# HunterJ-Lin/WSOVOD

Hardware: AMD Instinct MI355X
Metric: images/sec (512 proposals/img) WSR_18_DC5 fwd+bwd at 1/2/4/8 MI355X (higher is better)
Workload: dtype bf16 / fp16 + MX fp8 (the parity forward with the res4 / res5 convs and fc1 / fc2 on fp16 hi*hi + block-scaled e4m3 cross terms -- two v_mfma_f32_32x32x16_f16 + one v_mfma_scale_f32_32x32x64_f8f6f4 per 32x32x32 tile --, bf16x2 three-product forward elsewhere; plain bf16 backward; fp32 accumulation

## Files before the change

### include/wsovod_hip.h

```cpp
#ifndef WSOVOD_HIP_H_
#define WSOVOD_HIP_H_

#ifdef __cplusplus
extern "C" {
#endif

typedef void* wsovod_stream_t;

typedef enum {
  WSOVOD_OK = 0,
  WSOVOD_ERR_INVALID_ARGUMENT = 1,
  WSOVOD_ERR_HIP = 2,
  WSOVOD_ERR_UNSUPPORTED = 3
} wsovod_status;

typedef enum { WSOVOD_F32 = 0, WSOVOD_BF16 = 1, WSOVOD_BF16X2 = 2, WSOVOD_BF16X2P = 3, WSOVOD_F16MX = 4 } wsovod_dtype;
typedef enum { WSOVOD_NCHW = 0, WSOVOD_NHWC = 1 } wsovod_layout;

const char* wsovod_last_error(void);
int wsovod_abi_version(void);

typedef struct {
  const char* name;
  long long launches;
// ... 199 lines not shown
int wsovod_gemm_tn(const void* P, long long ldp, const void* Q, long long ldq, int Mred, int NI, int NJ, float* C,
                   long long ldc, float alpha, int accumulate, wsovod_stream_t stream);
int wsovod_gemm_tn_ex(const void* P, long long ldp, const void* Q, long long ldq, int q_dtype, int Mred, int NI, int NJ,
                      float* C, long long ldc, float alpha, int accumulate, wsovod_stream_t stream);
typedef struct wsovod_tn_sgd {
  float* param;
  float* momentum_buf;
  void* shadow;
  int shadow_is_bf16x2;
  float lr, weight_decay, momentum, grad_scale;
  const float* lr_dev;
  const unsigned char* mx_scale;
} wsovod_tn_sgd;
int wsovod_gemm_tn_sgd(const void* P, long long ldp, const void* Q, long long ldq, int q_dtype, int Mred, int NI, int NJ,
                       float alpha, const wsovod_tn_sgd* update, wsovod_stream_t stream);

int wsovod_f16mx_encode(const float* src, long long ld_src, int rows, int cols, int nseg, void* dst, long long ld_dst,
                        unsigned char* scales, wsovod_stream_t stream);
int wsovod_f16mx_encode_with(const float* src, long long ld_src, int rows, int cols, void* dst, long long ld_dst,
                             unsigned char* scales, const unsigned char* tensor_scale, wsovod_stream_t stream);
int wsovod_f16mx_from_bf16x2(const void* src, void* dst, long long n, wsovod_stream_t stream);
int wsovod_gemm_f16mx(const wsovod_gemm_desc* d, const unsigned char* a_scale, int a_segments, const unsigned char* b_scale,
                      int b_segments, void* c_bf16, long long ld_c_bf16, wsovod_stream_t stream);

typedef struct {
  int n_branch;
  int dil[4], pad[4];
  int shared_input;
} wsovod_conv_branches;
int wsovod_gemm_conv_branches(const wsovod_gemm_desc* d, const wsovod_conv_branches* br, wsovod_stream_t stream);
// ... 73 lines not shown
```

### wsovod_amd/_lib.py

```python
import ctypes as C
import os

import torch

_HERE = os.path.dirname(os.path.abspath(__file__))
LIB_PATH = os.path.join(_HERE, "lib", "libwsovod_hip.so")

F32, BF16, BF16X2, BF16X2P, F16MX = 0, 1, 2, 3, 4
NCHW, NHWC = 0, 1


class ConvGeom(C.Structure):
    _fields_ = [(n, C.c_int) for n in
                ("n_img", "H", "W", "Cin", "Ho", "Wo", "KH", "KW", "stride", "pad", "dil", "pool")]


class GemmDesc(C.Structure):
    _fields_ = [
        ("dtype_in", C.c_int), ("M", C.c_int), ("N", C.c_int), ("K", C.c_int),
        ("A", C.c_void_p), ("lda", C.c_longlong),
        ("B", C.c_void_p), ("ldb", C.c_longlong),
        ("C", C.c_void_p), ("ldc", C.c_longlong), ("dtype_c", C.c_int),
        ("Ct", C.c_void_p), ("ldct", C.c_longlong), ("dtype_ct", C.c_int),
        ("alpha", C.c_float),
# ... 74 lines not shown
    "wsovod_subsample_labels": [_P, _P, _P, _I, _I, _I, _I, _L, _P, _P],
    "wsovod_sgd_momentum_multi": [_P, _I, _F, _F, _P],
    "wsovod_grad_clip_workspace_floats": [_P, _I],
    "wsovod_grad_clip_coef": [_P, _I, _F, _F, _I, _P, _P, _P],
    "wsovod_roi_pool_workspace_bytes": [_I, _I, _I, _I, _I, _I, _I, _I, _I, _I],
    "wsovod_roi_pool_forward_ws": [_P, _I, _I, _P, _P, _I, _I, _I, _I, _I, _I, _I, _F, _P, _I, _P, _P, _P, _L, _P],
    "wsovod_roi_pool_forward_m2": [_P, _I, _I, _P, _P, _I, _I, _I, _I, _I, _I, _I, _F, _P, _I, _P, _P, _P, _L, _P],
    "wsovod_max2x2_gap_workspace_floats": [_I, _I, _I, _I, _I],
    "wsovod_max2x2_gap_nhwc": [_P, _I, _I, _I, _I, _I, _P, _P, _P, _P],
    "wsovod_pack_bf16_multi": [_P, _I, _P],
    "wsovod_sum_shards_bf16": [_P, _I, _L, _P, _P],
    "wsovod_format_rois": [_P, _P, _I, _I, _P, _P, _P, _P],
    "wsovod_gemm_tn": [_P, _L, _P, _L, _I, _I, _I, _P, _L, _F, _I, _P],
    "wsovod_gemm_tn_ex": [_P, _L, _P, _L, _I, _I, _I, _I, _P, _L, _F, _I, _P],
    "wsovod_gemm_tn_sgd": [_P, _L, _P, _L, _I, _I, _I, _I, _F, _P, _P],
    "wsovod_f16mx_encode": [_P, _L, _I, _I, _I, _P, _L, _P, _P],
    "wsovod_f16mx_encode_with": [_P, _L, _I, _I, _P, _L, _P, _P, _P],
    "wsovod_f16mx_from_bf16x2": [_P, _P, _L, _P],
    "wsovod_gemm_f16mx": [_P, _P, _I, _P, _I, _P, _L, _P],
    "wsovod_gemm_conv_branches": [C.POINTER(GemmDesc), C.POINTER(ConvBranches), _P],
    "wsovod_gemm_f16mx_conv_branches": [C.POINTER(GemmDesc), C.POINTER(ConvBranches), _P, _I, _P],
    "wsovod_mask_transpose_ex": [_P, _L, _I, _P, _L, _I, _I, _I, _F, _P, _L, _P, _L, _I, _P, _P],
    "wsovod_bf16x2_encode": [_P, _L, _I, _I, _P, _L, _P],
    "wsovod_bf16x2_decode": [_P, _L, _I, _I, _P, _L, _P],
    "wsovod_mask_bf16x2": [_P, _L, _P, _L, _I, _I, _I, _F, _P, _L, _P, _L, _P, _P],
    "wsovod_bf16x2_encode_t": [_P, _L, _I, _I, _P, _L, _P],
    "wsovod_f16mx_to_f32": [_P, _L, _I, _I, _P, _L, _P],
    "wsovod_f16mx_range": [_P, _L, _I, _I, _P, _P],
    "wsovod_stem_conv1_x2": [_P, _P, _P, _P, _I, _I, _I, _P, _P, _P, _P],
    "wsovod_nms_segments": [_P, _P, _P, _I, _I, _I, _F, _I, _P, _P, _P, _P],
# ... 104 lines not shown
```

### wsovod_amd/csrc/gemm_tn8.hip

```cpp
#include "gemm_common.h"
#include "f16mx.h"
#include <vector>

namespace wsovod_gemm {

namespace {

typedef __attribute__((ext_vector_type(4))) unsigned int u32x4;
typedef __attribute__((ext_vector_type(2))) unsigned int u32x2;

struct TnArgs {
  const char* P;
  const char* Q;
  long long ldp, ldq;
  int Mred, NI, NJ;
  float* C;
  long long ldc;
  float alpha;
  int accumulate;
  int tiles_i, tiles_j, group_m;
  int full_tiles, ksplit, slice_steps;
  float* partial;
#if defined(TN_STAMPS)
  float* dbg;
#endif
  int q_x2;
  float* mom;
  bf16_t* shadow;
  int shadow_x2;
  const unsigned char* mx_scale;
  float lr, wd, mu, gscale;
  const float* lr_dev;
  float* tail_buf;
  int bid_base;
};

template <int OFF>
__device__ __forceinline__ void tr_read_imm(__attribute__((ext_vector_type(2))) unsigned int& dst, unsigned addr) {
#if defined(__HIP_DEVICE_COMPILE__)
  asm volatile("ds_read_b64_tr_b16 %0, %1 offset:%2" : "=v"(dst) : "v"(addr), "n"(OFF));
#endif
}

template <int LEAN, bool SGD = false, bool TAILBUF = false>
__global__ __launch_bounds__(512) void gemm_tn8_kernel(const TnArgs p) {
  constexpr int BI = 256, BJ = 256, BK = 64;
  constexpr int OP_BYTES = 2 * BK * 256;
  constexpr int STEP_BYTES = 2 * OP_BYTES;
  constexpr int BUF_STRIDE = LEAN ? OP_BYTES : STEP_BYTES, OPQ_BASE = LEAN == 2 ? 2 * 5 * 8192 : LEAN ? 2 * OP_BYTES : OP_BYTES;
  constexpr int REG = 5 * 32 * 256;
  constexpr int SUB_STRIDE = LEAN == 2 ? REG : BK * 256;
  extern __shared__ __attribute__((aligned(16))) char smem[];

  int wg, slice = 0;
  const int bid = TAILBUF ? (int)blockIdx.x + p.bid_base : (int)blockIdx.x;
  {
    const int nwg = p.ksplit ? p.full_tiles : p.tiles_i * p.tiles_j;
    if (bid < nwg) {
      const int q = nwg >> 3, r = nwg & 7, xcd = bid & 7;
      wg = (xcd < r ? xcd * (q + 1) : r * (q + 1) + (xcd - r) * q) + (bid >> 3);
    } else {
      const int t = bid - nwg;
      wg = nwg + t / p.ksplit;
      slice = t - (t / p.ksplit) * p.ksplit;
    }
  }
  const bool sliced = p.ksplit && bid >= p.full_tiles;
  const int group_size = p.group_m * p.tiles_j;
  const int group_id = wg / group_size;
  const int first_i = group_id * p.group_m;
// ... 278 lines not shown
  if (sliced) {
    constexpr int SROW = 64;
    float* stg = (float*)smem + wave * (64 * SROW);
    const int cbase = j0 + wc * 64;
#pragma unroll
    for (int half = 0; half < 2; ++half) {
#pragma unroll
      for (int i = 0; i < 4; ++i)
#pragma unroll
        for (int j = 0; j < 4; ++j)
          *(f32x4*)(stg + (i * 16 + frow) * SROW + (((j * 4 + fq) ^ frow) << 2)) = acc[half * 4 + i][j] * p.alpha;
      __builtin_amdgcn_fence(__ATOMIC_RELEASE, "wavefront");
      __builtin_amdgcn_wave_barrier();
      const int rbase = i0 + wr * 128 + half * 64;
      const long long blk = (long long)(wr * 128 + half * 64) * 256 + wc * 64;
      float* dst = TAILBUF ? p.tail_buf + (long long)(wg - p.full_tiles) * 65536 + blk
                           : p.partial + ((long long)(wg - p.full_tiles) * p.ksplit + slice) * 65536 + blk;
      for (int row = 0; row < 64; ++row) {
        if (rbase + row >= p.NI) break;
        const float v = stg[row * SROW + ((((lane >> 2) ^ (row & 15)) << 2) | (lane & 3))];
        if (cbase + lane < p.NJ) {
          if constexpr (TAILBUF) unsafeAtomicAdd(dst + row * 256 + lane, v);
          else dst[row * 256 + lane] = v;
        }
      }
      __builtin_amdgcn_fence(__ATOMIC_ACQUIRE, "wavefront");
      __builtin_amdgcn_wave_barrier();
    }
    return;
  }
  if constexpr (SGD) {
    constexpr int SROW = 64;
    float* stg = (float*)smem + wave * (64 * SROW);
    const float lr = p.lr_dev ? *p.lr_dev : p.lr;
    const float ag = p.alpha, gs = p.gscale, mu = p.mu, wd = p.wd;
    const int mx_exp = p.shadow_x2 == 2 ? (int)*p.mx_scale - 127 : 0;
    const float mx_iq = __builtin_ldexpf(1.0f, -mx_exp), mx_il = __builtin_ldexpf(1.0f, -(mx_exp - 11));
    const int cbase = j0 + wc * 64;
    const int rsub = lane >> 4, c4 = (lane & 15) << 2;
#pragma unroll
    for (int half = 0; half < 2; ++half) {
#pragma unroll
      for (int i = 0; i < 4; ++i)
#pragma unroll
        for (int j = 0; j < 4; ++j)
          *(f32x4*)(stg + (i * 16 + frow) * SROW + (((j * 4 + fq) ^ frow) << 2)) = acc[half * 4 + i][j];
      __builtin_amdgcn_fence(__ATOMIC_RELEASE, "wavefront");
      __builtin_amdgcn_wave_barrier();
      const int rbase = i0 + wr * 128 + half * 64;
      if (cbase + c4 < p.NJ) {
#pragma unroll 4
        for (int it = 0; it < 16; ++it) {
          const int row = it * 4 + rsub;
          if (rbase + row >= p.NI) break;
          f32x4 gv = *(const f32x4*)(stg + row * SROW + ((((c4 >> 2)) ^ (row & 15)) << 2));
          const long long e = (long long)(rbase + row) * p.ldc + cbase + c4;
          f32x4 pv = __builtin_nontemporal_load((const f32x4*)(p.C + e));
          f32x4 bv = __builtin_nontemporal_load((const f32x4*)(p.mom + e));
          gv = gv * ag;
          gv = gv * gs;
          bv = mu * bv + (gv + wd * pv);
          pv -= lr * bv;
          __builtin_nontemporal_store(bv, (f32x4*)(p.mom + e));
          __builtin_nontemporal_store(pv, (f32x4*)(p.C + e));
          if (p.shadow && p.shadow_x2 == 2) {
            wsovod_mx::f16x4 h4;
            int q4, l4;
            wsovod_mx::mx_enc4(pv, mx_iq, mx_il, h4, q4, l4);
            char* grp = (char*)p.shadow + ((e >> 5) << 7);
            const int w = (int)(e & 31);
            *(wsovod_mx::f16x4*)(grp + 2 * w) = h4;
            *(int*)(grp + 64 + w) = q4;
            *(int*)(grp + 96 + w) = l4;
          } else if (p.shadow) {
            const bf16x4 hi = bf16x4{(bf16_t)pv[0], (bf16_t)pv[1], (bf16_t)pv[2], (bf16_t)pv[3]};
            if (p.shadow_x2) {
              bf16_t* q = p.shadow + ((e >> 5) << 6) + (e & 31);
              *(bf16x4*)q = hi;
              *(bf16x4*)(q + 32) = bf16x4{(bf16_t)(pv[0] - (float)hi[0]), (bf16_t)(pv[1] - (float)hi[1]),
                                          (bf16_t)(pv[2] - (float)hi[2]), (bf16_t)(pv[3] - (float)hi[3])};
            } else {
              *(bf16x4*)(p.shadow + e) = hi;
            }
          }
        }
      }
      __builtin_amdgcn_fence(__ATOMIC_ACQUIRE, "wavefront");
      __builtin_amdgcn_wave_barrier();
    }
    return;
  }
  const bool vec = (p.ldc & 3) == 0 && ((uintptr_t)p.C & 15) == 0 && j0 + BJ <= p.NJ;
#define WS_TN_ROW(I)                                                                                      \
  {                                                                                                       \
    const int ii = i0 + wr * 128 + (I) * 16 + frow;                                                       \
    if (ii < p.NI) {                                                                                      \
      float* crow = p.C + (long long)ii * p.ldc + j0 + wc * 64 + fq * 4;                                  \
// ... 34 lines not shown
    if (i >= p.NI) break;
    if (j >= p.NJ) continue;
    f32x4 acc = *(const f32x4*)(src + r * 256 + c4);
    for (int z = 1; z < nslices; ++z) acc += *(const f32x4*)(src + (long long)z * 65536 + r * 256 + c4);
    float* c = p.C + (long long)i * p.ldc + j;
    if (vec) {
      if (p.accumulate) acc += *(const f32x4*)c;
      *(f32x4*)c = acc;
    } else {
#pragma unroll
      for (int q = 0; q < 4; ++q) c[q] = p.accumulate ? c[q] + acc[q] : acc[q];
    }
  }
}

__global__ __launch_bounds__(256) void tn_sgd_tail_kernel(const TnArgs p) {
  const int wg = p.full_tiles + (blockIdx.x >> 4), part = blockIdx.x & 15;
  const int group_size = p.group_m * p.tiles_j;
  const int group_id = wg / group_size;
  const int first_i = group_id * p.group_m;
  const int gm = min(p.tiles_i - first_i, p.group_m);
  const int in_group = wg - group_id * group_size;
  const int i0 = (first_i + in_group % gm) * 256 + part * 16, j0 = (in_group / gm) * 256;
  const float* src = p.tail_buf + (long long)(wg - p.full_tiles) * 65536 + (long long)part * 16 * 256;
  const float lr = p.lr_dev ? *p.lr_dev : p.lr;
  const float gs = p.gscale, mu = p.mu, wd = p.wd;
  for (int e = threadIdx.x; e < 16 * 64; e += 256) {
    const int r = e >> 6, c4 = (e & 63) * 4;
    const int i = i0 + r, j = j0 + c4;
    if (i >= p.NI) break;
    if (j >= p.NJ) continue;
    f32x4 gv = *(const f32x4*)(src + r * 256 + c4);
    const long long q = (long long)i * p.ldc + j;
    f32x4 pv = *(const f32x4*)(p.C + q);
    f32x4 bv = *(const f32x4*)(p.mom + q);
    gv = gv * gs;
    bv = mu * bv + (gv + wd * pv);
    pv -= lr * bv;
    *(f32x4*)(p.mom + q) = bv;
    *(f32x4*)(p.C + q) = pv;
    if (p.shadow && p.shadow_x2 == 2) {
      const int mx_exp = (int)*p.mx_scale - 127;
      wsovod_mx::f16x4 h4;
      int q4, l4;
      wsovod_mx::mx_enc4(pv, __builtin_ldexpf(1.0f, -mx_exp), __builtin_ldexpf(1.0f, -(mx_exp - 11)), h4, q4, l4);
      char* grp = (char*)p.shadow + ((q >> 5) << 7);
      const int w = (int)(q & 31);
      *(wsovod_mx::f16x4*)(grp + 2 * w) = h4;
      *(int*)(grp + 64 + w) = q4;
      *(int*)(grp + 96 + w) = l4;
    } else if (p.shadow) {
      const bf16x4 hi = bf16x4{(bf16_t)pv[0], (bf16_t)pv[1], (bf16_t)pv[2], (bf16_t)pv[3]};
      if (p.shadow_x2) {
        bf16_t* d = p.shadow + ((q >> 5) << 6) + (q & 31);
        *(bf16x4*)d = hi;
        *(bf16x4*)(d + 32) = bf16x4{(bf16_t)(pv[0] - (float)hi[0]), (bf16_t)(pv[1] - (float)hi[1]),
                                    (bf16_t)(pv[2] - (float)hi[2]), (bf16_t)(pv[3] - (float)hi[3])};
      } else {
        *(bf16x4*)(p.shadow + q) = hi;
      }
    }
  }
}

}
}

static int tn_launch(const void* P, long long ldp, const void* Q, long long ldq, int q_dtype, int Mred, int NI, int NJ,
                     float* C, long long ldc, float alpha, int accumulate, const wsovod_tn_sgd* upd, wsovod_stream_t stream);

extern "C" int wsovod_gemm_tn_ex(const void* P, long long ldp, const void* Q, long long ldq, int q_dtype, int Mred, int NI,
                                 int NJ, float* C, long long ldc, float alpha, int accumulate, wsovod_stream_t stream) {
  return tn_launch(P, ldp, Q, ldq, q_dtype, Mred, NI, NJ, C, ldc, alpha, accumulate, nullptr, stream);
}

extern "C" int wsovod_gemm_tn_sgd(const void* P, long long ldp, const void* Q, long long ldq, int q_dtype, int Mred, int NI,
                                  int NJ, float alpha, const wsovod_tn_sgd* upd, wsovod_stream_t stream) {
  WS_CHECK_ARG(upd && upd->param && upd->momentum_buf, "wsovod_gemm_tn_sgd: null parameter / momentum buffer");
  WS_CHECK_ARG((((uintptr_t)upd->param | (uintptr_t)upd->momentum_buf) & 15) == 0 && ((uintptr_t)upd->shadow & 7) == 0,
               "wsovod_gemm_tn_sgd: parameter / momentum buffer must be 16-byte aligned (shadow: 8)");
  WS_CHECK_ARG(!upd->shadow || !upd->shadow_is_bf16x2 || NJ % 32 == 0,
               "wsovod_gemm_tn_sgd: a bf16x2 / f16mx shadow needs rows of whole 32-value groups");
  WS_CHECK_ARG(!upd->shadow || upd->shadow_is_bf16x2 != 2 || (upd->mx_scale && ((uintptr_t)upd->shadow & 15) == 0),
               "wsovod_gemm_tn_sgd: an f16mx shadow needs its per-tensor scale byte and 16-byte alignment");
  return tn_launch(P, ldp, Q, ldq, q_dtype, Mred, NI, NJ, upd->param, NJ, alpha, 2, upd, stream);
}

extern "C" int wsovod_gemm_tn(const void* P, long long ldp, const void* Q, long long ldq, int Mred, int NI, int NJ,
                              float* C, long long ldc, float alpha, int accumulate, wsovod_stream_t stream) {
  return wsovod_gemm_tn_ex(P, ldp, Q, ldq, WSOVOD_BF16, Mred, NI, NJ, C, ldc, alpha, accumulate, stream);
}

static int tn_launch(const void* P, long long ldp, const void* Q, long long ldq, int q_dtype, int Mred, int NI, int NJ,
                     float* C, long long ldc, float alpha, int accumulate, const wsovod_tn_sgd* upd, wsovod_stream_t stream) {
  using namespace wsovod_gemm;
  WS_CHECK_ARG(q_dtype == WSOVOD_BF16 || q_dtype == WSOVOD_BF16X2, "wsovod_gemm_tn: Q must be bf16 or bf16x2");
  const bool q_x2 = q_dtype == WSOVOD_BF16X2;
  WS_CHECK_ARG(!q_x2 || (NJ % 32 == 0 && ldq % 4 == 0), "wsovod_gemm_tn: a bf16x2 Q needs NJ a multiple of 32");
  if (q_x2) ldq *= 2;
  WS_CHECK_ARG(Mred >= 0 && NI >= 0 && NJ >= 0, "wsovod_gemm_tn: negative dimension");
  if (NI == 0 || NJ == 0) return WSOVOD_OK;
  WS_CHECK_ARG(P && Q && C, "wsovod_gemm_tn: null pointer");
  WS_CHECK_ARG((((uintptr_t)P | (uintptr_t)Q) & 15) == 0, "wsovod_gemm_tn: P/Q must be 16-byte aligned");
  WS_CHECK_ARG(ldp % 8 == 0 && ldq % 8 == 0 && NI % 8 == 0 && NJ % 8 == 0,
               "wsovod_gemm_tn: row strides and column counts must be multiples of 8 bf16 elements");
  WS_CHECK_ARG((long long)Mred * ldp * 2 < (1ll << 31) && (long long)Mred * ldq * 2 < (1ll << 31),
               "wsovod_gemm_tn: operand exceeds the 2 GiB buffer-addressing limit");
  TnArgs a;
  a.P = (const char*)P;
// ... 3 lines not shown
  a.Mred = Mred;
  a.NI = NI;
  a.NJ = NJ;
  a.C = C;
  a.ldc = ldc;
  a.alpha = alpha;
  a.accumulate = accumulate & 1;
  a.q_x2 = q_x2 ? 1 : 0;
  a.mom = nullptr;
  a.shadow = nullptr;
  a.shadow_x2 = 0;
  a.mx_scale = nullptr;
  a.lr = a.wd = a.mu = 0.f;
  a.gscale = 1.f;
  a.lr_dev = nullptr;
  a.tail_buf = nullptr;
  a.bid_base = 0;
  if (upd) {
    a.mom = upd->momentum_buf;
    a.shadow = (bf16_t*)upd->shadow;
    a.shadow_x2 = upd->shadow_is_bf16x2;
    a.mx_scale = upd->mx_scale;
    a.lr = upd->lr;
    a.wd = upd->weight_decay;
    a.mu = upd->momentum;
    a.gscale = upd->grad_scale;
    a.lr_dev = upd->lr_dev;
  }
#if defined(TN_STAMPS)
  a.dbg = getenv("WSOVOD_TN_DEBUG_PTR") ? (float*)strtoull(getenv("WSOVOD_TN_DEBUG_PTR"), nullptr, 16) : nullptr;
#endif
  a.tiles_i = ceil_div(NI, 256);
// ... 2 lines not shown
    const int run = std::max(1, a.tiles_i * a.tiles_j / 8);
    int g = 1;
    while ((g + 1) * (g + 1) <= run) ++g;
    a.group_m = std::max(1, std::min(std::min(g, 8), a.tiles_i));
  }
  static int slot_plain = wsovod::prof_slot("gemm_tn_bf16_256x256_tr");
  static int slot_sgd = wsovod::prof_slot("gemm_tn_bf16_256x256_tr_sgd");
  const int slot = upd ? slot_sgd : slot_plain;
  static bool attr_set = false;
  constexpr int lds_bytes = 2 * 2 * 2 * 64 * 256;
  if (!attr_set) {
    WS_CHECK_HIP(hipFuncSetAttribute((const void*)gemm_tn8_kernel<0>, hipFuncAttributeMaxDynamicSharedMemorySize, lds_bytes), "wsovod_gemm_tn: LDS opt-in");
    WS_CHECK_HIP(hipFuncSetAttribute((const void*)gemm_tn8_kernel<1>, hipFuncAttributeMaxDynamicSharedMemorySize, lds_bytes), "wsovod_gemm_tn: LDS opt-in");
    WS_CHECK_HIP(hipFuncSetAttribute((const void*)gemm_tn8_kernel<2>, hipFuncAttributeMaxDynamicSharedMemorySize, 160 * 1024), "wsovod_gemm_tn: LDS opt-in (160 KiB)");
    WS_CHECK_HIP(hipFuncSetAttribute((const void*)gemm_tn8_kernel<2, true>, hipFuncAttributeMaxDynamicSharedMemorySize, 160 * 1024), "wsovod_gemm_tn_sgd: LDS opt-in (160 KiB)");
    WS_CHECK_HIP(hipFuncSetAttribute((const void*)gemm_tn8_kernel<2, false, true>, hipFuncAttributeMaxDynamicSharedMemorySize, 160 * 1024), "wsovod_gemm_tn_sgd (tail): LDS opt-in (160 KiB)");
    attr_set = true;
  }
  hipStream_t s = (hipStream_t)stream;
  const double flops = 2.0 * Mred * NI * NJ;
  const double bytes = 2.0 * Mred * ((double)NI + NJ) + (upd ? (upd->shadow ? (upd->shadow_is_bf16x2 ? 20.0 : 18.0) : 16.0) : 4.0) * NI * NJ;
  wsovod::ProfScope prof(slot, s, flops, bytes);
  const int ntiles = a.tiles_i * a.tiles_j, cus = 256;
  const int tail = ntiles % cus, nk = ceil_div(Mred, 64);
  a.full_tiles = ntiles;
  a.ksplit = a.slice_steps = 0;
  a.accumulate = accumulate & 1;
  int grid = ntiles;
  if (!(accumulate & 2) && ntiles <= cus / 2 && nk >= 32) {
    const int S = std::min(std::min(8, cus / ntiles), nk / 16);
    if (S >= 2) {
      a.full_tiles = 0;
      a.ksplit = S;
      a.slice_steps = (ceil_div(nk, S) + 1) & ~1;
      grid = ntiles * S;
    }
  } else if (!(accumulate & 2) && ntiles > cus && tail > 0 && tail <= cus / 2 &&
             !(getenv("WSOVOD_TN_TAIL") && getenv("WSOVOD_TN_TAIL")[0] == '0')) {
    const int S = std::min(8, cus / tail);
    if (nk >= 8 * S) {
      a.full_tiles = ntiles - tail;
      a.ksplit = S;
      a.slice_steps = (ceil_div(nk, S) + 1) & ~1;
      grid = a.full_tiles + tail * S;
    }
  }
  a.partial = nullptr;
  if (a.ksplit && !upd) {
    static float* ws = nullptr;
    if (!ws) {
      hipStreamCaptureStatus cap = hipStreamCaptureStatusNone;
      if (s && hipStreamIsCapturing(s, &cap) == hipSuccess && cap != hipStreamCaptureStatusNone) {
        wsovod::set_error("wsovod_gemm_tn: the split-K workspace is allocated at the first split launch, not under stream "
                          "capture; run a split shape once outside the capture first");
        return WSOVOD_ERR_UNSUPPORTED;
      }
      if (hipMalloc((void**)&ws, (size_t)cus * 65536 * sizeof(float)) != hipSuccess) {
        ws = nullptr;
        wsovod::set_error("wsovod_gemm_tn: cannot allocate the split-K workspace");
        return WSOVOD_ERR_HIP;
      }
    }
    a.partial = ws;
  }
  static const int lean = getenv("WSOVOD_TN_LEAN") ? atoi(getenv("WSOVOD_TN_LEAN")) : 2;
  if (upd) {
    const bool want_tail = ntiles > cus && tail > 0 && tail <= cus / 2 &&
                           getenv("WSOVOD_TN_SGD_TAIL") && getenv("WSOVOD_TN_SGD_TAIL")[0] == '1';
    const int S = want_tail ? std::min(8, cus / tail) : 0;
    if (want_tail && S >= 2 && nk >= 8 * S) {
      static float* tb = nullptr;
      static size_t tb_bytes = 0;
      static std::vector<float*> retired;
      const size_t need = (size_t)tail * 65536 * sizeof(float);
      if (need > tb_bytes) {
        hipStreamCaptureStatus cap = hipStreamCaptureStatusNone;
        if (s && hipStreamIsCapturing(s, &cap) == hipSuccess && cap != hipStreamCaptureStatusNone) {
          wsovod::set_error("wsovod_gemm_tn_sgd: the tail scratch would have to grow under stream capture; run the shape once "
                            "outside the capture first");
          return WSOVOD_ERR_UNSUPPORTED;
        }
        float* fresh = nullptr;
        const size_t want = std::max(need, std::min<size_t>(2 * tb_bytes, (size_t)128 * 65536 * sizeof(float)));
        if (hipMalloc((void**)&fresh, want) != hipSuccess) {
          wsovod::set_error("wsovod_gemm_tn_sgd: cannot allocate the tail scratch");
          return WSOVOD_ERR_HIP;
        }
        if (tb) retired.push_back(tb);
        tb = fresh;
        tb_bytes = want;
      }
      a.tail_buf = tb;
      a.full_tiles = ntiles - tail;
      a.ksplit = S;
      a.slice_steps = (ceil_div(nk, S) + 1) & ~1;
      a.bid_base = a.full_tiles;
      WS_CHECK_HIP(hipMemsetAsync(tb, 0, need, s), "wsovod_gemm_tn_sgd: tail scratch");
      hipLaunchKernelGGL((gemm_tn8_kernel<2, true>), dim3(a.full_tiles), dim3(512), 160 * 1024, s, a);
      hipLaunchKernelGGL((gemm_tn8_kernel<2, false, true>), dim3(tail * S), dim3(512), 160 * 1024, s, a);
      hipLaunchKernelGGL(tn_sgd_tail_kernel, dim3(tail * 16), dim3(256), 0, s, a);
    } else {
      hipLaunchKernelGGL((gemm_tn8_kernel<2, true>), dim3(grid), dim3(512), 160 * 1024, s, a);
    }
  } else if (lean == 2)
    hipLaunchKernelGGL(gemm_tn8_kernel<2>, dim3(grid), dim3(512), 160 * 1024, s, a);
  else if (lean == 1)
    hipLaunchKernelGGL(gemm_tn8_kernel<1>, dim3(grid), dim3(512), lds_bytes, s, a);
  else
    hipLaunchKernelGGL(gemm_tn8_kernel<0>, dim3(grid), dim3(512), lds_bytes, s, a);
  if (a.partial) hipLaunchKernelGGL(tn_sum_slices_kernel, dim3((ntiles - a.full_tiles) * 16), dim3(256), 0, s, a);
  WS_CHECK_LAUNCH("wsovod_gemm_tn");
  return WSOVOD_OK;
}
```

### wsovod_amd/engine/trainer.py

```python
import gc as _gc
import os
import warnings
import weakref

import torch
import torch.distributed as dist

from ..layers import hip_ops as H
from ..layers import operand_cache


class HipSGD(torch.optim.Optimizer):

    def __init__(self, params, lr, momentum=0.0, weight_decay=0.0, clip=None):
        super().__init__(params, dict(lr=lr, momentum=momentum, weight_decay=weight_decay))
        self.grad_scale = 1.0
        if clip is not None and (clip[0] not in ("full_model", "norm", "value") or not clip[1] > 0.0):
            raise ValueError(f"HipSGD: clip must be (full_model | norm | value, positive value), got {clip!r}")
        self.clip = clip
        self.last_clip_coef = None
        self.lr_device = None

    @torch.no_grad()
    def step(self, closure=None):
# ... 12 lines not shown
                lr = group["lr"] if self.lr_device is None else self.lr_device[p]
                by_momentum.setdefault(group["momentum"], []).append(
                    (p.data, g, state["momentum_buffer"], shadow, lr, group["weight_decay"],
                     getattr(p, "_used_flag", None), p, fmt))
        if self.clip is not None and self.clip[0] == "full_model" and len(by_momentum) > 1:
            raise NotImplementedError("HipSGD: full-model clipping needs one momentum value for all parameter groups")
        for mu, entries in by_momentum.items():
            self.last_clip_coef = H.sgd_momentum_multi([e[:7] for e in entries], mu, grad_scale=self.grad_scale,
                                                       clip=self.clip)
            for e in entries:
                operand_cache.wrote(e[7], e[8])


class _FusedUpdate:

    def __init__(self, optimizer, param, max_rows):
        self.opt = weakref.proxy(optimizer)
        self.param = weakref.ref(param)
        self.max_rows = int(max_rows)
        self.group_index = self._find_group(optimizer, param)
        self.calls = 0
        self.armed = False

    @staticmethod
    def _find_group(optimizer, param):
        return next(i for i, g in enumerate(optimizer.param_groups) if any(q is param for q in g["params"]))

    @property
    def group(self):
        groups, p = self.opt.param_groups, self.param()
        g = groups[self.group_index] if self.group_index < len(groups) else None
        if g is None or not any(q is p for q in g["params"]):
            self.group_index = self._find_group(self.opt, p)
            g = groups[self.group_index]
        return g

    def wants(self, rows):
        p = self.param()
        return self.armed and p is not None and rows <= self.max_rows and p.grad is None \
            and getattr(p, "_wire_grad", None) is None \
            and self.opt.clip is None and getattr(p, "_used_flag", None) is None

    def __call__(self, dA, x, q_x2):
        p, opt, g = self.param(), self.opt, self.group
        state = opt.state[p]
        if "momentum_buffer" not in state:
            state["momentum_buffer"] = torch.zeros_like(p, memory_format=torch.contiguous_format)
        fmt, shadow = operand_cache.refreshable(p)
        lr = g["lr"] if opt.lr_device is None else opt.lr_device[p]
        H.gemm_tn_sgd(dA, x, p.data, state["momentum_buffer"], shadow, lr, g["weight_decay"], g["momentum"],
                      grad_scale=opt.grad_scale, q_x2=q_x2)
        operand_cache.wrote(p, fmt)
        self.calls += 1
        return True
# ... 354 lines not shown
            raise ValueError(f"iter_size must be >= 1, got {iter_size}")
        if self.iter:
            for m in model.modules():
                if hasattr(m, "set_step"):
                    m.set_step(self.iter)
        for p in self.params:
            p._wire_grad = None
        if self.exchange and grad_wire == "bf16" and self.params and self.iter_size == 1:
            self._setup_early_exchange()
        self._fused = []
        if (not self.exchange and self.iter_size == 1 and isinstance(optimizer, HipSGD) and optimizer.clip is None
                and self.params and os.environ.get("WSOVOD_FUSED_SGD", "1") != "0"):
            for big in sorted(self.params, key=lambda q: -q.numel()):
                if big.dim() == 2 and big.is_cuda and big.is_contiguous() and big.numel() >= (1 << 24) and big.shape[1] % 32 == 0:
                    self._fused.append(big)
                    big._fused_update = _FusedUpdate(optimizer, big, int(os.environ.get("WSOVOD_FUSED_SGD_ROWS", "4096")))
        self._hooks = []
        if hasattr(model, "register_state_dict_pre_hook"):
            self._hooks.append(model.register_state_dict_pre_hook(lambda *_a, **_k: self.synchronize()))
        if hasattr(optimizer, "register_state_dict_pre_hook"):
            self._hooks.append(optimizer.register_state_dict_pre_hook(lambda *_a, **_k: self.synchronize()))
        for obj in (model, optimizer):
            if hasattr(obj, "register_load_state_dict_pre_hook"):
                self._hooks.append(obj.register_load_state_dict_pre_hook(lambda *_a, **_k: self.synchronize()))
            if hasattr(obj, "register_load_state_dict_post_hook"):
                self._hooks.append(obj.register_load_state_dict_post_hook(lambda *_a, **_k: self._drop_graphs()))
        if isinstance(optimizer, HipSGD):
            optimizer.grad_scale = 1.0 / self.world
        ref = weakref.ref(self)

        def _pre_inference():
# ... 455 lines not shown
```

### wsovod_amd/layers/hip_ops.py

```python
import ctypes as C
import contextlib
import os
import threading

import torch

from .. import _lib
from .._lib import BF16, BF16X2, BF16X2P, F16MX, F32, NCHW, NHWC, ConvBranches, GemmDesc, check, dtype_code, lib, ptr, require_gpu, stream
from . import carrier, operand_cache
from .precision import mx_active, mx_mode, x2_active, x3_active, x3_mode


_CONST_CACHE = {}


class _ConstOverride(threading.local):
    table = None


_OVERRIDE = _ConstOverride()


class const_override:
    def __init__(self, table):
# ... 1202 lines not shown
    split_tail = split_tail and not DETERMINISTIC
    assert P.dtype == torch.bfloat16 and Q.dtype == (torch.float32 if q_x2 else torch.bfloat16) and P.shape[0] == Q.shape[0]
    Mred, NI, NJ = P.shape[0], P.shape[1], Q.shape[1]
    if out is None:
        out = torch.empty((NI, NJ), dtype=torch.float32, device=P.device)
    limit = GEMM_TN_MAX_OPERAND_BYTES // (2 * max(_ld(P), _ld(Q) * (2 if q_x2 else 1), 1))
    step = max(64, limit // 64 * 64) if Mred > limit else max(Mred, 1)
    for r0 in range(0, max(Mred, 1), step):
        r1 = min(Mred, r0 + step)
        check(lib().wsovod_gemm_tn_ex(ptr(P[r0:r1]), _ld(P), ptr(Q[r0:r1]), _ld(Q), BF16X2 if q_x2 else BF16, r1 - r0, NI,
                                      NJ, ptr(out), _ld(out), C.c_float(alpha),
                                      int(bool(accumulate) or r0 > 0) | (0 if split_tail else 2), stream()), "gemm_tn")
    return out


def gemm_tn_sgd(P, Q, param, momentum_buf, shadow, lr, weight_decay, momentum, grad_scale=1.0, alpha=1.0, q_x2=False):
    from .._lib import TnSgd

    mx_byte = None
    if isinstance(shadow, tuple):
        shadow, mx_byte = shadow
    require_gpu(P, Q, param, momentum_buf, shadow, mx_byte)
    carrier.refuse("gemm_tn_sgd", (P, Q), reads=(MX,))
    assert P.dtype == torch.bfloat16 and Q.dtype == (torch.float32 if q_x2 else torch.bfloat16) and P.shape[0] == Q.shape[0]
    Mred, NI, NJ = P.shape[0], P.shape[1], Q.shape[1]
    if tuple(param.shape) != (NI, NJ) or not param.is_contiguous() or param.dtype != torch.float32 \
            or momentum_buf.shape != param.shape or not momentum_buf.is_contiguous() or momentum_buf.dtype != torch.float32:
        raise RuntimeError("wsovod_hip gemm_tn_sgd: param / momentum buffer must be contiguous fp32 (NI, NJ)")
    if 2 * Mred * max(_ld(P), _ld(Q) * (2 if q_x2 else 1)) >= GEMM_TN_MAX_OPERAND_BYTES:
        raise RuntimeError("wsovod_hip gemm_tn_sgd: the reduction does not fit one launch (the fused update needs the "
                           "finished sum of a tile)")
    u = TnSgd()
    u.param, u.momentum_buf = param.data_ptr(), momentum_buf.data_ptr()
    u.shadow = shadow.data_ptr() if shadow is not None else None
    u.shadow_is_bf16x2 = 2 if mx_byte is not None else int(shadow is not None and shadow.dtype == torch.float32)
    u.mx_scale = mx_byte.data_ptr() if mx_byte is not None else None
    if shadow is not None and (shadow.numel() != param.numel() or not shadow.is_contiguous()):
        raise RuntimeError("wsovod_hip gemm_tn_sgd: the shadow must be a contiguous copy of the parameter")
    if torch.is_tensor(lr):
        require_gpu(lr)
        u.lr, u.lr_dev = 0.0, lr.data_ptr()
    else:
        u.lr, u.lr_dev = float(lr), None
    u.weight_decay, u.momentum, u.grad_scale = float(weight_decay), float(momentum), float(grad_scale)
    check(lib().wsovod_gemm_tn_sgd(ptr(P), _ld(P), ptr(Q), _ld(Q), BF16X2 if q_x2 else BF16, Mred, NI, NJ, C.c_float(alpha),
                                   C.byref(u), stream()), "gemm_tn_sgd")


def sgd_momentum_multi(entries, momentum, grad_scale=1.0, clip=None):
    from .._lib import SgdTensor

    if not entries:
        return
    arr = (SgdTensor * len(entries))()
    coef = None
    for d, e in zip(arr, entries):
        p, g, b, sh, lr, wd = e[:6]
        used = e[6] if len(e) > 6 else None
        mx_byte = None
        if isinstance(sh, tuple):
            sh, mx_byte = sh
# ... 57 lines not shown
```

Measured before the change: 1429.

## Fuse split-K tail reduction and SGD update into the TN gemm via arrival counters

Replaces the opt-in three-launch tail path (atomics into a zeroed scratch, then a separate update kernel) with a single SGD gemm launch. Tail tiles are split along K, each slice writes its partial to the workspace, and the last slice to arrive, found through a per-tile atomic ticket counter, sums the slices and applies the momentum update and shadow encoding. The split tail is now on by default, the fused-update row limit rises from 4096 to 16384, and the whole-tile epilogue batches its parameter and momentum loads. The price is a last-arriver fence protocol with counters that reset themselves, and reuse of the shared split-K workspace, which assumes no more than 128 tail tiles.

```diff
diff --git a/include/wsovod_hip.h b/include/wsovod_hip.h
--- a/include/wsovod_hip.h
+++ b/include/wsovod_hip.h
@@ -237,6 +237,9 @@
 } wsovod_tn_sgd;
 int wsovod_gemm_tn_sgd(const void* P, long long ldp, const void* Q, long long ldq, int q_dtype, int Mred, int NI, int NJ,
                        float alpha, const wsovod_tn_sgd* update, wsovod_stream_t stream);
+#define WSOVOD_TN_SGD_WHOLE_TILES 1
+int wsovod_gemm_tn_sgd_ex(const void* P, long long ldp, const void* Q, long long ldq, int q_dtype, int Mred, int NI, int NJ,
+                          float alpha, const wsovod_tn_sgd* update, int flags, wsovod_stream_t stream);
 
 int wsovod_f16mx_encode(const float* src, long long ld_src, int rows, int cols, int nseg, void* dst, long long ld_dst,
                         unsigned char* scales, wsovod_stream_t stream);
diff --git a/wsovod_amd/_lib.py b/wsovod_amd/_lib.py
--- a/wsovod_amd/_lib.py
+++ b/wsovod_amd/_lib.py
@@ -112,6 +112,7 @@
     "wsovod_gemm_tn": [_P, _L, _P, _L, _I, _I, _I, _P, _L, _F, _I, _P],
     "wsovod_gemm_tn_ex": [_P, _L, _P, _L, _I, _I, _I, _I, _P, _L, _F, _I, _P],
     "wsovod_gemm_tn_sgd": [_P, _L, _P, _L, _I, _I, _I, _I, _F, _P, _P],
+    "wsovod_gemm_tn_sgd_ex": [_P, _L, _P, _L, _I, _I, _I, _I, _F, _P, _I, _P],
     "wsovod_f16mx_encode": [_P, _L, _I, _I, _I, _P, _L, _P, _P],
     "wsovod_f16mx_encode_with": [_P, _L, _I, _I, _P, _L, _P, _P, _P],
     "wsovod_f16mx_from_bf16x2": [_P, _P, _L, _P],
diff --git a/wsovod_amd/csrc/gemm_tn8.hip b/wsovod_amd/csrc/gemm_tn8.hip
--- a/wsovod_amd/csrc/gemm_tn8.hip
+++ b/wsovod_amd/csrc/gemm_tn8.hip
@@ -31,9 +31,47 @@
   const unsigned char* mx_scale;
   float lr, wd, mu, gscale;
   const float* lr_dev;
-  float* tail_buf;
-  int bid_base;
+  int* tail_cnt;
 };
+
+typedef __attribute__((__vector_size__(4 * sizeof(unsigned)))) unsigned tn_b128;
+
+#define WS_TN_SGD_CONSTS(p)                                                               \
+  const float k_lr = (p).lr_dev ? *(p).lr_dev : (p).lr;                                   \
+  const int k_mx_exp = (p).shadow_x2 == 2 ? (int)*(p).mx_scale - 127 : 0;                 \
+  const float k_mx_iq = __builtin_ldexpf(1.0f, -k_mx_exp), k_mx_il = __builtin_ldexpf(1.0f, -(k_mx_exp - 11))
+#define WS_TN_SGD_K(p) k_lr, (p).gscale, (p).mu, (p).wd, k_mx_iq, k_mx_il
+__device__ __forceinline__ void tn_sgd_update4(const TnArgs& p, float lr, float gs, float mu, float wd, float mx_iq, float mx_il,
+                                               long long e, f32x4 gv, f32x4 pv, f32x4 bv) {
+  const f32x4 gg = gv * gs;
+#pragma unroll
+  for (int c = 0; c < 4; ++c) {
+    bv[c] = __builtin_fmaf(mu, bv[c], __builtin_fmaf(wd, pv[c], gg[c]));
+    pv[c] = __builtin_fmaf(-lr, bv[c], pv[c]);
+  }
+  __builtin_nontemporal_store(bv, (f32x4*)(p.mom + e));
+  __builtin_nontemporal_store(pv, (f32x4*)(p.C + e));
+  if (p.shadow && p.shadow_x2 == 2) {
+    wsovod_mx::f16x4 h4;
+    int q4, l4;
+    wsovod_mx::mx_enc4(pv, mx_iq, mx_il, h4, q4, l4);
+    char* grp = (char*)p.shadow + ((e >> 5) << 7);
+    const int w = (int)(e & 31);
+    *(wsovod_mx::f16x4*)(grp + 2 * w) = h4;
+    *(int*)(grp + 64 + w) = q4;
+    *(int*)(grp + 96 + w) = l4;
+  } else if (p.shadow) {
+    const bf16x4 hi = bf16x4{(bf16_t)pv[0], (bf16_t)pv[1], (bf16_t)pv[2], (bf16_t)pv[3]};
+    if (p.shadow_x2) {
+      bf16_t* q = p.shadow + ((e >> 5) << 6) + (e & 31);
+      *(bf16x4*)q = hi;
+      *(bf16x4*)(q + 32) = bf16x4{(bf16_t)(pv[0] - (float)hi[0]), (bf16_t)(pv[1] - (float)hi[1]),
+                                  (bf16_t)(pv[2] - (float)hi[2]), (bf16_t)(pv[3] - (float)hi[3])};
+    } else {
+      *(bf16x4*)(p.shadow + e) = hi;
+    }
+  }
+}
 
 template <int OFF>
 __device__ __forceinline__ void tr_read_imm(__attribute__((ext_vector_type(2))) unsigned int& dst, unsigned addr) {
@@ -42,7 +80,7 @@
 #endif
 }
 
-template <int LEAN, bool SGD = false, bool TAILBUF = false>
+template <int LEAN, bool SGD = false>
 __global__ __launch_bounds__(512) void gemm_tn8_kernel(const TnArgs p) {
   constexpr int BI = 256, BJ = 256, BK = 64;
   constexpr int OP_BYTES = 2 * BK * 256;
@@ -53,7 +91,7 @@
   extern __shared__ __attribute__((aligned(16))) char smem[];
 
   int wg, slice = 0;
-  const int bid = TAILBUF ? (int)blockIdx.x + p.bid_base : (int)blockIdx.x;
+  const int bid = (int)blockIdx.x;
   {
     const int nwg = p.ksplit ? p.full_tiles : p.tiles_i * p.tiles_j;
     if (bid < nwg) {
@@ -362,28 +400,71 @@
       __builtin_amdgcn_wave_barrier();
       const int rbase = i0 + wr * 128 + half * 64;
       const long long blk = (long long)(wr * 128 + half * 64) * 256 + wc * 64;
-      float* dst = TAILBUF ? p.tail_buf + (long long)(wg - p.full_tiles) * 65536 + blk
-                           : p.partial + ((long long)(wg - p.full_tiles) * p.ksplit + slice) * 65536 + blk;
+      float* dst = p.partial + ((long long)(wg - p.full_tiles) * p.ksplit + slice) * 65536 + blk;
       for (int row = 0; row < 64; ++row) {
         if (rbase + row >= p.NI) break;
         const float v = stg[row * SROW + ((((lane >> 2) ^ (row & 15)) << 2) | (lane & 3))];
         if (cbase + lane < p.NJ) {
-          if constexpr (TAILBUF) unsafeAtomicAdd(dst + row * 256 + lane, v);
-          else dst[row * 256 + lane] = v;
+          dst[row * 256 + lane] = v;
         }
       }
       __builtin_amdgcn_fence(__ATOMIC_ACQUIRE, "wavefront");
       __builtin_amdgcn_wave_barrier();
+    }
+    if constexpr (SGD) {
+      const int t = wg - p.full_tiles;
+      int* last = (int*)(smem + 128 * 1024);
+#if defined(__HIP_DEVICE_COMPILE__)
+      asm volatile("s_waitcnt vmcnt(0)" ::: "memory");
+#endif
+      __syncthreads();
+      if (tid == 0) {
+        __threadfence();
+        const int arrivals = min(p.ksplit, (nk_all + p.slice_steps - 1) / p.slice_steps);
+        const int ticket = __hip_atomic_fetch_add(p.tail_cnt + t, 1, __ATOMIC_RELAXED, __HIP_MEMORY_SCOPE_AGENT);
+        const int is_last = ticket == arrivals - 1;
+        if (is_last) {
+          __builtin_amdgcn_fence(__ATOMIC_ACQUIRE, "agent");
+#if defined(__HIP_DEVICE_COMPILE__)
+          asm volatile("s_waitcnt vmcnt(0)" ::: "memory");
+#endif
+        }
+        *last = is_last;
+      }
+      __syncthreads();
+      if (!*last) return;
+      WS_TN_SGD_CONSTS(p);
+      const int nsl = min(p.ksplit, (nk_all + p.slice_steps - 1) / p.slice_steps);
+      const __amdgpu_buffer_rsrc_t rs = __builtin_amdgcn_make_buffer_rsrc(
+          (void*)(p.partial + (long long)t * p.ksplit * 65536), 0, p.ksplit * 65536 * 4, 0x00020000);
+      const int c4 = (tid & 63) << 2, r8 = tid >> 6;
+      if (j0 + c4 < p.NJ) {
+        for (int pass = 0; pass < 32; ++pass) {
+          const int r = pass * 8 + r8;
+          if (i0 + r >= p.NI) break;
+          const long long e = (long long)(i0 + r) * p.ldc + j0 + c4;
+          const f32x4 pv = __builtin_nontemporal_load((const f32x4*)(p.C + e));
+          const f32x4 bv = __builtin_nontemporal_load((const f32x4*)(p.mom + e));
+          f32x4 sl[8];
+#pragma unroll
+          for (int z = 0; z < 8; ++z)
+            sl[z] = __builtin_bit_cast(f32x4, __builtin_amdgcn_raw_buffer_load_b128(rs, (r * 256 + c4) * 4, min(z, nsl - 1) * 262144, 16));
+          f32x4 gv = sl[0];
+#pragma unroll
+          for (int z = 1; z < 8; ++z)
+            if (z < nsl) gv += sl[z];
+          tn_sgd_update4(p, WS_TN_SGD_K(p), e, gv, pv, bv);
+        }
+      }
+      if (tid == 0) __hip_atomic_store(p.tail_cnt + t, 0, __ATOMIC_RELAXED, __HIP_MEMORY_SCOPE_AGENT);
     }
     return;
   }
   if constexpr (SGD) {
     constexpr int SROW = 64;
     float* stg = (float*)smem + wave * (64 * SROW);
-    const float lr = p.lr_dev ? *p.lr_dev : p.lr;
-    const float ag = p.alpha, gs = p.gscale, mu = p.mu, wd = p.wd;
-    const int mx_exp = p.shadow_x2 == 2 ? (int)*p.mx_scale - 127 : 0;
-    const float mx_iq = __builtin_ldexpf(1.0f, -mx_exp), mx_il = __builtin_ldexpf(1.0f, -(mx_exp - 11));
+    WS_TN_SGD_CONSTS(p);
+    const float ag = p.alpha;
     const int cbase = j0 + wc * 64;
     const int rsub = lane >> 4, c4 = (lane & 15) << 2;
 #pragma unroll
@@ -397,38 +478,24 @@
       __builtin_amdgcn_wave_barrier();
       const int rbase = i0 + wr * 128 + half * 64;
       if (cbase + c4 < p.NJ) {
-#pragma unroll 4
-        for (int it = 0; it < 16; ++it) {
-          const int row = it * 4 + rsub;
-          if (rbase + row >= p.NI) break;
-          f32x4 gv = *(const f32x4*)(stg + row * SROW + ((((c4 >> 2)) ^ (row & 15)) << 2));
-          const long long e = (long long)(rbase + row) * p.ldc + cbase + c4;
-          f32x4 pv = __builtin_nontemporal_load((const f32x4*)(p.C + e));
-          f32x4 bv = __builtin_nontemporal_load((const f32x4*)(p.mom + e));
-          gv = gv * ag;
-          gv = gv * gs;
-          bv = mu * bv + (gv + wd * pv);
-          pv -= lr * bv;
-          __builtin_nontemporal_store(bv, (f32x4*)(p.mom + e));
-          __builtin_nontemporal_store(pv, (f32x4*)(p.C + e));
-          if (p.shadow && p.shadow_x2 == 2) {
-            wsovod_mx::f16x4 h4;
-            int q4, l4;
-            wsovod_mx::mx_enc4(pv, mx_iq, mx_il, h4, q4, l4);
-            char* grp = (char*)p.shadow + ((e >> 5) << 7);
-            const int w = (int)(e & 31);
-            *(wsovod_mx::f16x4*)(grp + 2 * w) = h4;
-            *(int*)(grp + 64 + w) = q4;
-            *(int*)(grp + 96 + w) = l4;
-          } else if (p.shadow) {
-            const bf16x4 hi = bf16x4{(bf16_t)pv[0], (bf16_t)pv[1], (bf16_t)pv[2], (bf16_t)pv[3]};
-            if (p.shadow_x2) {
-              bf16_t* q = p.shadow + ((e >> 5) << 6) + (e & 31);
-              *(bf16x4*)q = hi;
-              *(bf16x4*)(q + 32) = bf16x4{(bf16_t)(pv[0] - (float)hi[0]), (bf16_t)(pv[1] - (float)hi[1]),
-                                          (bf16_t)(pv[2] - (float)hi[2]), (bf16_t)(pv[3] - (float)hi[3])};
-            } else {
-              *(bf16x4*)(p.shadow + e) = hi;
+        constexpr int NB = 8;
+        for (int it0 = 0; it0 < 16; it0 += NB) {
+          f32x4 pv[NB], bv[NB];
+#pragma unroll
+          for (int u = 0; u < NB; ++u) {
+            const int row = min(rbase + (it0 + u) * 4 + rsub, p.NI - 1);
+            const long long e = (long long)row * p.ldc + cbase + c4;
+            pv[u] = __builtin_nontemporal_load((const f32x4*)(p.C + e));
+            bv[u] = __builtin_nontemporal_load((const f32x4*)(p.mom + e));
+          }
+#pragma unroll
+          for (int u = 0; u < NB; ++u) {
+            const int row = (it0 + u) * 4 + rsub;
+            if (rbase + row < p.NI) {
+              const long long e = (long long)(rbase + row) * p.ldc + cbase + c4;
+              f32x4 gv = *(const f32x4*)(stg + row * SROW + ((((c4 >> 2)) ^ (row & 15)) << 2));
+              gv = gv * ag;
+              tn_sgd_update4(p, WS_TN_SGD_K(p), e, gv, pv[u], bv[u]);
             }
           }
         }
@@ -493,68 +560,25 @@
   }
 }
 
-__global__ __launch_bounds__(256) void tn_sgd_tail_kernel(const TnArgs p) {
-  const int wg = p.full_tiles + (blockIdx.x >> 4), part = blockIdx.x & 15;
-  const int group_size = p.group_m * p.tiles_j;
-  const int group_id = wg / group_size;
-  const int first_i = group_id * p.group_m;
-  const int gm = min(p.tiles_i - first_i, p.group_m);
-  const int in_group = wg - group_id * group_size;
-  const int i0 = (first_i + in_group % gm) * 256 + part * 16, j0 = (in_group / gm) * 256;
-  const float* src = p.tail_buf + (long long)(wg - p.full_tiles) * 65536 + (long long)part * 16 * 256;
-  const float lr = p.lr_dev ? *p.lr_dev : p.lr;
-  const float gs = p.gscale, mu = p.mu, wd = p.wd;
-  for (int e = threadIdx.x; e < 16 * 64; e += 256) {
-    const int r = e >> 6, c4 = (e & 63) * 4;
-    const int i = i0 + r, j = j0 + c4;
-    if (i >= p.NI) break;
-    if (j >= p.NJ) continue;
-    f32x4 gv = *(const f32x4*)(src + r * 256 + c4);
-    const long long q = (long long)i * p.ldc + j;
-    f32x4 pv = *(const f32x4*)(p.C + q);
-    f32x4 bv = *(const f32x4*)(p.mom + q);
-    gv = gv * gs;
-    bv = mu * bv + (gv + wd * pv);
-    pv -= lr * bv;
-    *(f32x4*)(p.mom + q) = bv;
-    *(f32x4*)(p.C + q) = pv;
-    if (p.shadow && p.shadow_x2 == 2) {
-      const int mx_exp = (int)*p.mx_scale - 127;
-      wsovod_mx::f16x4 h4;
-      int q4, l4;
-      wsovod_mx::mx_enc4(pv, __builtin_ldexpf(1.0f, -mx_exp), __builtin_ldexpf(1.0f, -(mx_exp - 11)), h4, q4, l4);
-      char* grp = (char*)p.shadow + ((q >> 5) << 7);
-      const int w = (int)(q & 31);
-      *(wsovod_mx::f16x4*)(grp + 2 * w) = h4;
-      *(int*)(grp + 64 + w) = q4;
-      *(int*)(grp + 96 + w) = l4;
-    } else if (p.shadow) {
-      const bf16x4 hi = bf16x4{(bf16_t)pv[0], (bf16_t)pv[1], (bf16_t)pv[2], (bf16_t)pv[3]};
-      if (p.shadow_x2) {
-        bf16_t* d = p.shadow + ((q >> 5) << 6) + (q & 31);
-        *(bf16x4*)d = hi;
-        *(bf16x4*)(d + 32) = bf16x4{(bf16_t)(pv[0] - (float)hi[0]), (bf16_t)(pv[1] - (float)hi[1]),
-                                    (bf16_t)(pv[2] - (float)hi[2]), (bf16_t)(pv[3] - (float)hi[3])};
-      } else {
-        *(bf16x4*)(p.shadow + q) = hi;
-      }
-    }
-  }
-}
-
 }
 }
 
 static int tn_launch(const void* P, long long ldp, const void* Q, long long ldq, int q_dtype, int Mred, int NI, int NJ,
-                     float* C, long long ldc, float alpha, int accumulate, const wsovod_tn_sgd* upd, wsovod_stream_t stream);
+                     float* C, long long ldc, float alpha, int accumulate, const wsovod_tn_sgd* upd, int upd_flags,
+                     wsovod_stream_t stream);
 
 extern "C" int wsovod_gemm_tn_ex(const void* P, long long ldp, const void* Q, long long ldq, int q_dtype, int Mred, int NI,
                                  int NJ, float* C, long long ldc, float alpha, int accumulate, wsovod_stream_t stream) {
-  return tn_launch(P, ldp, Q, ldq, q_dtype, Mred, NI, NJ, C, ldc, alpha, accumulate, nullptr, stream);
+  return tn_launch(P, ldp, Q, ldq, q_dtype, Mred, NI, NJ, C, ldc, alpha, accumulate, nullptr, 0, stream);
 }
 
 extern "C" int wsovod_gemm_tn_sgd(const void* P, long long ldp, const void* Q, long long ldq, int q_dtype, int Mred, int NI,
                                   int NJ, float alpha, const wsovod_tn_sgd* upd, wsovod_stream_t stream) {
+  return wsovod_gemm_tn_sgd_ex(P, ldp, Q, ldq, q_dtype, Mred, NI, NJ, alpha, upd, 0, stream);
+}
+
+extern "C" int wsovod_gemm_tn_sgd_ex(const void* P, long long ldp, const void* Q, long long ldq, int q_dtype, int Mred, int NI,
+                                     int NJ, float alpha, const wsovod_tn_sgd* upd, int flags, wsovod_stream_t stream) {
   WS_CHECK_ARG(upd && upd->param && upd->momentum_buf, "wsovod_gemm_tn_sgd: null parameter / momentum buffer");
   WS_CHECK_ARG((((uintptr_t)upd->param | (uintptr_t)upd->momentum_buf) & 15) == 0 && ((uintptr_t)upd->shadow & 7) == 0,
                "wsovod_gemm_tn_sgd: parameter / momentum buffer must be 16-byte aligned (shadow: 8)");
@@ -562,7 +586,7 @@
                "wsovod_gemm_tn_sgd: a bf16x2 / f16mx shadow needs rows of whole 32-value groups");
   WS_CHECK_ARG(!upd->shadow || upd->shadow_is_bf16x2 != 2 || (upd->mx_scale && ((uintptr_t)upd->shadow & 15) == 0),
                "wsovod_gemm_tn_sgd: an f16mx shadow needs its per-tensor scale byte and 16-byte alignment");
-  return tn_launch(P, ldp, Q, ldq, q_dtype, Mred, NI, NJ, upd->param, NJ, alpha, 2, upd, stream);
+  return tn_launch(P, ldp, Q, ldq, q_dtype, Mred, NI, NJ, upd->param, NJ, alpha, 2, upd, flags, stream);
 }
 
 extern "C" int wsovod_gemm_tn(const void* P, long long ldp, const void* Q, long long ldq, int Mred, int NI, int NJ,
@@ -571,7 +595,8 @@
 }
 
 static int tn_launch(const void* P, long long ldp, const void* Q, long long ldq, int q_dtype, int Mred, int NI, int NJ,
-                     float* C, long long ldc, float alpha, int accumulate, const wsovod_tn_sgd* upd, wsovod_stream_t stream) {
+                     float* C, long long ldc, float alpha, int accumulate, const wsovod_tn_sgd* upd, int upd_flags,
+                     wsovod_stream_t stream) {
   using namespace wsovod_gemm;
   WS_CHECK_ARG(q_dtype == WSOVOD_BF16 || q_dtype == WSOVOD_BF16X2, "wsovod_gemm_tn: Q must be bf16 or bf16x2");
   const bool q_x2 = q_dtype == WSOVOD_BF16X2;
@@ -605,8 +630,7 @@
   a.lr = a.wd = a.mu = 0.f;
   a.gscale = 1.f;
   a.lr_dev = nullptr;
-  a.tail_buf = nullptr;
-  a.bid_base = 0;
+  a.tail_cnt = nullptr;
   if (upd) {
     a.mom = upd->momentum_buf;
     a.shadow = (bf16_t*)upd->shadow;
@@ -639,7 +663,6 @@
     WS_CHECK_HIP(hipFuncSetAttribute((const void*)gemm_tn8_kernel<1>, hipFuncAttributeMaxDynamicSharedMemorySize, lds_bytes), "wsovod_gemm_tn: LDS opt-in");
     WS_CHECK_HIP(hipFuncSetAttribute((const void*)gemm_tn8_kernel<2>, hipFuncAttributeMaxDynamicSharedMemorySize, 160 * 1024), "wsovod_gemm_tn: LDS opt-in (160 KiB)");
     WS_CHECK_HIP(hipFuncSetAttribute((const void*)gemm_tn8_kernel<2, true>, hipFuncAttributeMaxDynamicSharedMemorySize, 160 * 1024), "wsovod_gemm_tn_sgd: LDS opt-in (160 KiB)");
-    WS_CHECK_HIP(hipFuncSetAttribute((const void*)gemm_tn8_kernel<2, false, true>, hipFuncAttributeMaxDynamicSharedMemorySize, 160 * 1024), "wsovod_gemm_tn_sgd (tail): LDS opt-in (160 KiB)");
     attr_set = true;
   }
   hipStream_t s = (hipStream_t)stream;
@@ -670,9 +693,22 @@
       grid = a.full_tiles + tail * S;
     }
   }
+  static const int lean = getenv("WSOVOD_TN_LEAN") ? atoi(getenv("WSOVOD_TN_LEAN")) : 2;
+  if (upd) {
+    const bool want_tail = ntiles > cus && tail > 0 && tail <= cus / 2 && !(upd_flags & WSOVOD_TN_SGD_WHOLE_TILES) &&
+                           !(getenv("WSOVOD_TN_SGD_TAIL") && getenv("WSOVOD_TN_SGD_TAIL")[0] == '0');
+    const int S = want_tail ? std::min(8, cus / tail) : 0;
+    if (want_tail && S >= 2 && nk >= 8 * S) {
+      a.full_tiles = ntiles - tail;
+      a.ksplit = S;
+      a.slice_steps = (ceil_div(nk, S) + 1) & ~1;
+      grid = a.full_tiles + tail * S;
+    }
+  }
   a.partial = nullptr;
-  if (a.ksplit && !upd) {
+  if (a.ksplit) {
     static float* ws = nullptr;
+    constexpr size_t ws_bytes = (size_t)cus * 65536 * sizeof(float), cnt_bytes = 128 * sizeof(int);
     if (!ws) {
       hipStreamCaptureStatus cap = hipStreamCaptureStatusNone;
       if (s && hipStreamIsCapturing(s, &cap) == hipSuccess && cap != hipStreamCaptureStatusNone) {
@@ -680,60 +716,30 @@
                           "capture; run a split shape once outside the capture first");
         return WSOVOD_ERR_UNSUPPORTED;
       }
-      if (hipMalloc((void**)&ws, (size_t)cus * 65536 * sizeof(float)) != hipSuccess) {
-        ws = nullptr;
+      float* fresh = nullptr;
+      if (hipMalloc((void**)&fresh, ws_bytes + cnt_bytes) != hipSuccess) {
         wsovod::set_error("wsovod_gemm_tn: cannot allocate the split-K workspace");
         return WSOVOD_ERR_HIP;
       }
+      if (hipMemsetAsync((char*)fresh + ws_bytes, 0, cnt_bytes, s) != hipSuccess || hipStreamSynchronize(s) != hipSuccess) {
+        (void)hipFree(fresh);
+        wsovod::set_error("wsovod_gemm_tn: cannot clear the arrival counters of the split-K workspace");
+        return WSOVOD_ERR_HIP;
+      }
+      ws = fresh;
     }
     a.partial = ws;
-  }
-  static const int lean = getenv("WSOVOD_TN_LEAN") ? atoi(getenv("WSOVOD_TN_LEAN")) : 2;
+    a.tail_cnt = (int*)((char*)ws + ws_bytes);
+  }
   if (upd) {
-    const bool want_tail = ntiles > cus && tail > 0 && tail <= cus / 2 &&
-                           getenv("WSOVOD_TN_SGD_TAIL") && getenv("WSOVOD_TN_SGD_TAIL")[0] == '1';
-    const int S = want_tail ? std::min(8, cus / tail) : 0;
-    if (want_tail && S >= 2 && nk >= 8 * S) {
-      static float* tb = nullptr;
-      static size_t tb_bytes = 0;
-      static std::vector<float*> retired;
-      const size_t need = (size_t)tail * 65536 * sizeof(float);
-      if (need > tb_bytes) {
-        hipStreamCaptureStatus cap = hipStreamCaptureStatusNone;
-        if (s && hipStreamIsCapturing(s, &cap) == hipSuccess && cap != hipStreamCaptureStatusNone) {
-          wsovod::set_error("wsovod_gemm_tn_sgd: the tail scratch would have to grow under stream capture; run the shape once "
-                            "outside the capture first");
-          return WSOVOD_ERR_UNSUPPORTED;
-        }
-        float* fresh = nullptr;
-        const size_t want = std::max(need, std::min<size_t>(2 * tb_bytes, (size_t)128 * 65536 * sizeof(float)));
-        if (hipMalloc((void**)&fresh, want) != hipSuccess) {
-          wsovod::set_error("wsovod_gemm_tn_sgd: cannot allocate the tail scratch");
-          return WSOVOD_ERR_HIP;
-        }
-        if (tb) retired.push_back(tb);
-        tb = fresh;
-        tb_bytes = want;
-      }
-      a.tail_buf = tb;
-      a.full_tiles = ntiles - tail;
-      a.ksplit = S;
-      a.slice_steps = (ceil_div(nk, S) + 1) & ~1;
-      a.bid_base = a.full_tiles;
-      WS_CHECK_HIP(hipMemsetAsync(tb, 0, need, s), "wsovod_gemm_tn_sgd: tail scratch");
-      hipLaunchKernelGGL((gemm_tn8_kernel<2, true>), dim3(a.full_tiles), dim3(512), 160 * 1024, s, a);
-      hipLaunchKernelGGL((gemm_tn8_kernel<2, false, true>), dim3(tail * S), dim3(512), 160 * 1024, s, a);
-      hipLaunchKernelGGL(tn_sgd_tail_kernel, dim3(tail * 16), dim3(256), 0, s, a);
-    } else {
-      hipLaunchKernelGGL((gemm_tn8_kernel<2, true>), dim3(grid), dim3(512), 160 * 1024, s, a);
-    }
+    hipLaunchKernelGGL((gemm_tn8_kernel<2, true>), dim3(grid), dim3(512), 160 * 1024, s, a);
   } else if (lean == 2)
     hipLaunchKernelGGL(gemm_tn8_kernel<2>, dim3(grid), dim3(512), 160 * 1024, s, a);
   else if (lean == 1)
     hipLaunchKernelGGL(gemm_tn8_kernel<1>, dim3(grid), dim3(512), lds_bytes, s, a);
   else
     hipLaunchKernelGGL(gemm_tn8_kernel<0>, dim3(grid), dim3(512), lds_bytes, s, a);
-  if (a.partial) hipLaunchKernelGGL(tn_sum_slices_kernel, dim3((ntiles - a.full_tiles) * 16), dim3(256), 0, s, a);
+  if (a.partial && !upd) hipLaunchKernelGGL(tn_sum_slices_kernel, dim3((ntiles - a.full_tiles) * 16), dim3(256), 0, s, a);
   WS_CHECK_LAUNCH("wsovod_gemm_tn");
   return WSOVOD_OK;
 }
diff --git a/wsovod_amd/engine/trainer.py b/wsovod_amd/engine/trainer.py
--- a/wsovod_amd/engine/trainer.py
+++ b/wsovod_amd/engine/trainer.py
@@ -50,6 +50,8 @@
 
 class _FusedUpdate:
 
+    WHOLE_TILE_ROWS = 4096
+
     def __init__(self, optimizer, param, max_rows):
         self.opt = weakref.proxy(optimizer)
         self.param = weakref.ref(param)
@@ -73,7 +75,8 @@
 
     def wants(self, rows):
         p = self.param()
-        return self.armed and p is not None and rows <= self.max_rows and p.grad is None \
+        max_rows = min(self.max_rows, self.WHOLE_TILE_ROWS) if H.DETERMINISTIC else self.max_rows
+        return self.armed and p is not None and rows <= max_rows and p.grad is None \
             and getattr(p, "_wire_grad", None) is None \
             and self.opt.clip is None and getattr(p, "_used_flag", None) is None
 
@@ -458,7 +461,7 @@
             for big in sorted(self.params, key=lambda q: -q.numel()):
                 if big.dim() == 2 and big.is_cuda and big.is_contiguous() and big.numel() >= (1 << 24) and big.shape[1] % 32 == 0:
                     self._fused.append(big)
-                    big._fused_update = _FusedUpdate(optimizer, big, int(os.environ.get("WSOVOD_FUSED_SGD_ROWS", "4096")))
+                    big._fused_update = _FusedUpdate(optimizer, big, int(os.environ.get("WSOVOD_FUSED_SGD_ROWS", "16384")))
         self._hooks = []
         if hasattr(model, "register_state_dict_pre_hook"):
             self._hooks.append(model.register_state_dict_pre_hook(lambda *_a, **_k: self.synchronize()))
diff --git a/wsovod_amd/layers/hip_ops.py b/wsovod_amd/layers/hip_ops.py
--- a/wsovod_amd/layers/hip_ops.py
+++ b/wsovod_amd/layers/hip_ops.py
@@ -1240,7 +1240,8 @@
     return out
 
 
-def gemm_tn_sgd(P, Q, param, momentum_buf, shadow, lr, weight_decay, momentum, grad_scale=1.0, alpha=1.0, q_x2=False):
+def gemm_tn_sgd(P, Q, param, momentum_buf, shadow, lr, weight_decay, momentum, grad_scale=1.0, alpha=1.0, q_x2=False,
+                split_tail=True):
     from .._lib import TnSgd
 
     mx_byte = None
@@ -1269,8 +1270,9 @@
     else:
         u.lr, u.lr_dev = float(lr), None
     u.weight_decay, u.momentum, u.grad_scale = float(weight_decay), float(momentum), float(grad_scale)
-    check(lib().wsovod_gemm_tn_sgd(ptr(P), _ld(P), ptr(Q), _ld(Q), BF16X2 if q_x2 else BF16, Mred, NI, NJ, C.c_float(alpha),
-                                   C.byref(u), stream()), "gemm_tn_sgd")
+    whole = 0 if split_tail and not DETERMINISTIC else 1
+    check(lib().wsovod_gemm_tn_sgd_ex(ptr(P), _ld(P), ptr(Q), _ld(Q), BF16X2 if q_x2 else BF16, Mred, NI, NJ,
+                                      C.c_float(alpha), C.byref(u), whole, stream()), "gemm_tn_sgd")
 
 
 def sgd_momentum_multi(entries, momentum, grad_scale=1.0, clip=None):
```

Result: no change. 1432 (median of 6 runs) (+0.3%).
